# korrawe/harp

Hardware: AMD Instinct MI355X
Metric: render+loss+backward+Adam frames/sec, 512x512 MANO hand mesh (higher is better)
Workload: dtype f32; 1 GPU; C3/C4: 256-frame 512x512 sequence, subdivided MANO hand 3093v/6152f/3327uv, self-shadow, coarse+appearance terms (displacement+texture stage, VGG excluded), dense Adam; global_batch=32, sequence_frames=256, hipgraph=True

## Files before the change

### harp_amd/csrc/shade.hip

```cpp
#include "shade_common.h"

namespace {

#ifndef SHADE_TEX_SLOTS
#define SHADE_TEX_SLOTS 512
#endif
#ifndef SHADE_VTX_SLOTS
#define SHADE_VTX_SLOTS 256
#endif
#ifndef SHADE_ACC_T
#define SHADE_ACC_T double
#endif
#ifndef SHADE_OCC
#define SHADE_OCC 3
#endif
constexpr int kTexSlots = SHADE_TEX_SLOTS, kVtxSlots = SHADE_VTX_SLOTS;
constexpr int kZlW = 32, kZlH = 24;
constexpr int kTexRows = 512;
#ifndef SHADE_PRERED
#define SHADE_PRERED 19
#endif
template <int SLOTS>
__device__ __forceinline__ int sort_slots_by_row(const int* __restrict__ keys, int width, int ylo, int yhi, int* s_box, int* s_hist,
                                                 int* s_order, int* s_wsum) {
// ... 229 lines not shown
      for (int ii = -1; ii <= 1; ++ii)
        for (int jj = -1; jj <= 1; ++jj, ++k) {
          const int yy = min(max(g.iy + ii, 0), S - 1), xx = min(max(g.ix + jj, 0), S - 1);
          tapo[k] = yy * S + xx;
          sg[k] = sigmoidf((A.zl[(size_t)b * S * S + tapo[k]] - aa) * 1000.0f);
          acc += sg[k];
        }
      g.vis = acc * (1.0f / 9.0f);
    }
    const V3 amb = ld(col), dfc = ld(col + 3), spc = ld(col + 6);
    const V3 lightc = mk(amb.x + dfc.x * cosang * g.vis, amb.y + dfc.y * cosang * g.vis, amb.z + dfc.z * cosang * g.vis);
    const V3 c = mk(lightc.x * g.texel.x + spc.x, lightc.y * g.texel.y + spc.y, lightc.z * g.texel.z + spc.z);
    const float zpix = b0 * g.t.z0 + b1 * g.t.z1 + b2 * g.t.z2;
    const float zinv = (100.0f - zpix) * (1.0f / 99.0f);
    const float zmax = fmaxf(zinv, 1e-10f);
    const float wnum = __expf((zinv - zmax) * 1e4f);
    const float delta = fmaxf(__expf((1e-10f - zmax) * 1e4f), 1e-10f);
    const float denom = wnum + delta;
    if (!BWD) {
      const float rden = rcp(denom);
      out_rgb[0] = (wnum * c.x + delta * A.bg[0]) * rden;
      out_rgb[1] = (wnum * c.y + delta * A.bg[1]) * rden;
      out_rgb[2] = (wnum * c.z + delta * A.bg[2]) * rden;
      if (A.rgb) { float* r = A.rgb + o * 3; r[0] = out_rgb[0]; r[1] = out_rgb[1]; r[2] = out_rgb[2]; }
    } else {
      const float wk = wnum * rcp(denom);
      if (fused_loss) {
        const float rden = rcp(denom);
        const float o3[3] = {(wnum * c.x + delta * A.bg[0]) * rden, (wnum * c.y + delta * A.bg[1]) * rden, (wnum * c.z + delta * A.bg[2]) * rden};
        const float wl = A.l1_w[0] * A.l1_inv * l1_m;
        float gq[3];
#pragma unroll
        for (int ch = 0; ch < 3; ++ch) {
          const float d = o3[ch] * l1_m - A.l1_target[l1_to * 3 + ch] * l1_m;
          racc[16] += fabsf(d);
          gq[ch] = wl * (float)((d > 0.f) - (d < 0.f));
        }
        gc = mk(gq[0], gq[1], gq[2]);
      }
      const V3 g_c = gc * wk;
      const V3 g_tex = mk(g_c.x * lightc.x, g_c.y * lightc.y, g_c.z * lightc.z);
      const V3 g_lc = mk(g_c.x * g.texel.x, g_c.y * g.texel.y, g_c.z * g.texel.z);
      racc[0] += g_lc.x; racc[1] += g_lc.y; racc[2] += g_lc.z;
      racc[3] += g_lc.x * cosang * g.vis; racc[4] += g_lc.y * cosang * g.vis; racc[5] += g_lc.z * cosang * g.vis;
      racc[6] += g_c.x; racc[7] += g_c.y; racc[8] += g_c.z;
      const float g_dv = g_lc.x * dfc.x + g_lc.y * dfc.y + g_lc.z * dfc.z;
      const float g_vis = g_dv * cosang;
      const float g_cos = (g.cosr > 0.f) ? g_dv * g.vis : 0.f;
      float gu = 0.f, gv = 0.f;
      V3 g_m_keep = mk(0.f, 0.f, 0.f);
      gu += dot(g_tex, tdx) * (float)(A.Wt - 1);
      gv += dot(g_tex, tdy) * -(float)(A.Ht - 1);
      V3 g_p = mk(0.f, 0.f, 0.f);
      const V3 g_nn = g.lhat * g_cos, g_lhat = g.nn * g_cos;
      V3 g_ldir = (g.llen > 1e-6f) ? (g_lhat - g.lhat * dot(g.lhat, g_lhat)) * rcp(g.llen) : g_lhat * 1e6f;
      racc[9] += g_ldir.x; racc[10] += g_ldir.y; racc[11] += g_ldir.z;
      g_p = g_p - g_ldir;
      V3 g_nfin = (g.lnh > 1e-6f) ? (g_nn - g.nn * dot(g.nn, g_nn)) * rcp(g.lnh) : g_nn * 1e6f;
      V3 g_n = g_nfin;
      if (A.nmap) {
        const V3 g_np = (g.lnp > 1e-12f) ? (g_nfin - g.nhat * dot(g.nhat, g_nfin)) * rcp(g.lnp) : g_nfin * 1e12f;
        const V3 g_m = mk(-dot(g.tu, g_np), -dot(g.tv, g_np), dot(g.n, g_np));
        g_m_keep = g_m;
        gu += dot(g_m, mdx) * (float)(A.Wt - 1);
        gv += dot(g_m, mdy) * -(float)(A.Ht - 1);
        const V3 g_tu = g_np * (-g.m.x), g_tv = g_np * (-g.m.y);
        g_n = g_np * g.m.z;
        const float x = g.n.x, y = g.n.y, s = g.s, a = g.a;
        const float g_b = s * g_tu.y + g_tv.x;
        const float g_a = s * x * x * g_tu.x + y * y * g_tv.y + g_b * x * y;
        g_n.x += 2.f * s * x * a * g_tu.x - s * g_tu.z + g_b * y * a;
        g_n.y += 2.f * y * a * g_tv.y - g_tv.z + g_b * x * a;
        g_n.z += g_a * a * a;
      }
      if (!(A.debug_skip & 1)) {
        const float ax = 1.f - g.bs.wx, ay = 1.f - g.bs.wy;
        const float cw[4] = {ax * ay, g.bs.wx * ay, ax * g.bs.wy, g.bs.wx * g.bs.wy};
        const int cx[4] = {g.bs.x0, g.bs.x0 + 1, g.bs.x0, g.bs.x0 + 1}, cy[4] = {g.bs.y0, g.bs.y0, g.bs.y0 + 1, g.bs.y0 + 1};
        const bool do_t = A.g_tex != nullptr, do_n = (A.nmap != nullptr) && (A.g_nmap != nullptr);
#pragma unroll
        for (int k = 0; k < 4; ++k) {
          if (cx[k] >= A.Wt || cy[k] >= A.Ht || cw[k] == 0.f) continue;
          const int key = cy[k] * A.Wt + cx[k];
          tb_y0 = min(tb_y0, cy[k]); tb_y1 = max(tb_y1, cy[k]);
          const int slot = s_tex.find(key);
          const float vals[6] = {g_tex.x * cw[k], g_tex.y * cw[k], g_tex.z * cw[k], g_m_keep.x * cw[k], g_m_keep.y * cw[k], g_m_keep.z * cw[k]};
          if (slot >= 0) {
#pragma unroll
            for (int c = 0; c < 3; ++c) { if (do_t) s_tex.add(slot, c, vals[c]); if (do_n) s_tex.add(slot, 3 + c, vals[3 + c]); }
          } else {
#pragma unroll
            for (int c = 0; c < 3; ++c) {
              if (do_t) atomicAdd(A.g_tex + (size_t)key * 3 + c, vals[c]);
              if (do_n) atomicAdd(A.g_nmap + (size_t)key * 3 + c, vals[3 + c]);
            }
          }
        }
      }
      if (A.zl) {
        float g_zq = 0.f;
        for (int k = 0; k < 9; ++k) {
          const float d = g_vis * (1.0f / 9.0f) * sg[k] * (1.0f - sg[k]) * 1000.0f;
          if (d != 0.f) {
            zd[BWD ? k : 0] = d;
            g_zq -= d;
          }
        }
        zix = g.ix; ziy = g.iy;
        const float* R = A.light_R + 9 * b;
        g_p = g_p + mk(R[2], R[5], R[8]) * g_zq;
        racc[12] += g.p.x * g_zq; racc[13] += g.p.y * g_zq; racc[14] += g.p.z * g_zq;
        racc[15] += g_zq;
      }
      float gb0 = dot(v0, g_p) + dot(n0, g_n) + uv0x * gu + uv0y * gv;
      float gb1 = dot(v1, g_p) + dot(n1, g_n) + uv1x * gu + uv1y * gv;
      float gb2 = dot(v2, g_p) + dot(n2, g_n) + uv2x * gu + uv2y * gv;
      float gnd[9] = {0.f, 0.f, 0.f, 0.f, 0.f, 0.f, 0.f, 0.f, 0.f};
      bary_bwd(g.t, px, py, g.br, gb0, gb1, gb2, gnd);
      const float bw[3] = {b0, b1, b2};
      vidx[0] = g.i0; vidx[1] = g.i1; vidx[2] = g.i2;
#pragma unroll
      for (int k = 0; k < 3; ++k) {
        vsc[9 * k + 0] = g_p.x * bw[k]; vsc[9 * k + 1] = g_p.y * bw[k]; vsc[9 * k + 2] = g_p.z * bw[k];
        vsc[9 * k + 3] = g_n.x * bw[k]; vsc[9 * k + 4] = g_n.y * bw[k]; vsc[9 * k + 5] = g_n.z * bw[k];
        vsc[9 * k + 6] = gnd[3 * k]; vsc[9 * k + 7] = gnd[3 * k + 1]; vsc[9 * k + 8] = gnd[3 * k + 2];
      }
    }
  }
  if (BWD && A.zl && A.g_zl && !(A.debug_skip & 4)) {
    if (threadIdx.x == 0) { s_zbox[0] = 0x7fffffff; s_zbox[1] = 0x7fffffff; }
    for (int i = threadIdx.x; i < kZlW * kZlH; i += 256) s_zwin[i] = 0.0;
    __syncthreads();
    const bool has = zix > -0x40000000;
    int mx = has ? min(max(zix - 1, 0), S - 1) : 0x7fffffff, my = has ? min(max(ziy - 1, 0), S - 1) : 0x7fffffff;
#pragma unroll
    for (int o2 = 32; o2 >= 1; o2 >>= 1) { mx = min(mx, __shfl_xor(mx, o2)); my = min(my, __shfl_xor(my, o2)); }
    if (lane == 0 && mx != 0x7fffffff) { atomicMin(&s_zbox[0], mx); atomicMin(&s_zbox[1], my); }
    __syncthreads();
    const int x0 = s_zbox[0], y0 = s_zbox[1];
    float* gz = A.g_zl + (size_t)b * S * S;
    const int znt = (S + 15) >> 4;
    if (has) {
#pragma unroll
      for (int r = 0; r < 3; ++r) {
        const int yy = min(max(ziy + r - 1, 0), S - 1);
#pragma unroll
        for (int c = 0; c < 3; ++c) {
          const float d = zd[BWD ? 3 * r + c : 0];
          if (d == 0.f) continue;
          const int xx = min(max(zix + c - 1, 0), S - 1);
          const int wx = xx - x0, wy = yy - y0;
          if (wx < kZlW && wy < kZlH) atomicAdd(&s_zwin[wy * kZlW + wx], (double)d);
          else {
            atomicAdd(gz + yy * S + xx, d);
            if (A.g_zl_tiles) A.g_zl_tiles[((size_t)b * znt + (yy >> 4)) * znt + (xx >> 4)] = 1;
          }
        }
      }
    }
    __syncthreads();
    if (x0 != 0x7fffffff) {
      for (int i = threadIdx.x; i < kZlW * kZlH; i += 256) {
        const double v = s_zwin[i];
        if (v != 0.0) {
          atomicAdd(gz + (size_t)(y0 + i / kZlW) * S + x0 + (i % kZlW), (float)v);
          if (A.g_zl_tiles) A.g_zl_tiles[((size_t)b * znt + ((y0 + i / kZlW) >> 4)) * znt + ((x0 + i % kZlW) >> 4)] = 1;
        }
      }
    }
  }
  if (BWD && !(A.debug_skip & 8)) {
    bool alive = act;
    merge_same_face<27, SHADE_PRERED>(vsc, act ? f : -1, alive, lane);
    if (alive) {
      float* gvb = A.g_verts + (size_t)b * V * 3;
      float* gnb = A.g_vnormals + (size_t)b * V * 3;
      float* gdb = A.g_ndc + (size_t)b * V * 3;
#pragma unroll
      for (int k = 0; k < 3; ++k) {
        const int slot = s_acc.find(vidx[k]);
        if (slot >= 0) {
#pragma unroll
          for (int c = 0; c < 9; ++c) s_acc.add(slot, c, vsc[9 * k + c]);
        } else {
#pragma unroll
          for (int c = 0; c < 3; ++c) {
            atomicAdd(gvb + 3 * vidx[k] + c, vsc[9 * k + c]); atomicAdd(gnb + 3 * vidx[k] + c, vsc[9 * k + 3 + c]);
            atomicAdd(gdb + 3 * vidx[k] + c, vsc[9 * k + 6 + c]);
          }
        }
      }
    }
  }
  if (!BWD && A.l1_target) {
    float acc = 0.f;
    if (in_img) {
      const size_t to = ((size_t)A.l1_fid[b] * S + yi) * S + xi;
      const float m = A.l1_mask ? A.l1_mask[to] : 1.f;
      const float wk = A.l1_w[0] * A.l1_inv * m;
      if (m != 0.f) {
#pragma unroll
        for (int ch = 0; ch < 3; ++ch) {
          const float d = out_rgb[ch] * m - A.l1_target[to * 3 + ch] * m;
          acc += fabsf(d);
          if (f >= 0) A.l1_grad[o * 3 + ch] = wk * ((d > 0.f) - (d < 0.f));
        }
      } else if (f >= 0) {
        A.l1_grad[o * 3] = 0.f; A.l1_grad[o * 3 + 1] = 0.f; A.l1_grad[o * 3 + 2] = 0.f;
      }
    }
    const float sum = block_sum_256(acc, s_red);
    if (threadIdx.x == 0 && sum != 0.f) atomicAdd(A.l1_loss, sum * A.l1_inv);
  }
  }
  if (BWD && fused_loss) {
    const float sum = block_sum_256(racc[16], s_red + 16);
    if (threadIdx.x == 0 && sum != 0.f) atomicAdd(A.l1_loss, sum * A.l1_inv);
  }
  if (BWD) {
#pragma unroll
    for (int k = 0; k < 16; ++k) {
      const float s = wave_sum(racc[k]);
      if (lane == 0 && s != 0.f) atomicAdd(&s_red[k], s);
    }
    __syncthreads();
    if (threadIdx.x < 16) {
      const float s = s_red[threadIdx.x];
      const int k = threadIdx.x;
      if (s != 0.f) {
        if (k < 9) { if (A.g_colors) atomicAdd(A.g_colors + k, s); }
        else if (k < 12) { if (A.g_light_pos) atomicAdd(A.g_light_pos + 3 * b + (k - 9), s); }
        else if (k < 15) { if (A.g_light_R) atomicAdd(A.g_light_R + 9 * b + 3 * (k - 12) + 2, s); }
        else if (A.g_light_T) atomicAdd(A.g_light_T + 3 * b + 2, s);
      }
    }
    float* gvb = A.g_verts + (size_t)b * V * 3;
    float* gnb = A.g_vnormals + (size_t)b * V * 3;
    float* gdb = A.g_ndc + (size_t)b * V * 3;
    for (int i = threadIdx.x; i < kVtxSlots; i += 256) {
      const int v = s_acc.key[i];
      if (v < 0 || (A.debug_skip & 32)) continue;
#pragma unroll
      for (int c = 0; c < 3; ++c) {
        const float a0 = (float)s_acc.val[i][c], a1 = (float)s_acc.val[i][3 + c], a2 = (float)s_acc.val[i][6 + c];
        if (a0 != 0.f) atomicAdd(gvb + 3 * v + c, a0);
        if (a1 != 0.f) atomicAdd(gnb + 3 * v + c, a1);
        if (a2 != 0.f) atomicAdd(gdb + 3 * v + c, a2);
      }
    }
    __shared__ int s_box[2];
    __shared__ int s_wsum[4];
    static_assert(sizeof(double) * kZlW * kZlH >= sizeof(int) * (kTexRows + kTexSlots), "window too small for the sort scratch");
    int* s_hist = (int*)s_zwin;
    int* s_order = s_hist + kTexRows;
    if (!(A.debug_skip & 16)) {
      const int total = sort_slots_by_row<kTexSlots>(s_tex.key, A.Wt, tb_y0, tb_y1, s_box, s_hist, s_order, s_wsum);
      if (total >= 0) {
        for (int i = threadIdx.x; i < total * 3; i += 256) {
          const int e = i / 3, c = i - 3 * e;
          const int slot = s_order[e];
          const int key = s_tex.key[slot];
          const float a0 = (float)s_tex.val[slot][c], a1 = (float)s_tex.val[slot][3 + c];
          if (a0 != 0.f) atomicAdd(A.g_tex + (size_t)key * 3 + c, a0);
          if (a1 != 0.f) atomicAdd(A.g_nmap + (size_t)key * 3 + c, a1);
        }
      } else {
        for (int i = threadIdx.x; i < kTexSlots; i += 256) {
          const int key = s_tex.key[i];
          if (key < 0) continue;
#pragma unroll
          for (int c = 0; c < 3; ++c) {
            const float a0 = (float)s_tex.val[i][c], a1 = (float)s_tex.val[i][3 + c];
            if (a0 != 0.f) atomicAdd(A.g_tex + (size_t)key * 3 + c, a0);
            if (a1 != 0.f) atomicAdd(A.g_nmap + (size_t)key * 3 + c, a1);
          }
        }
      }
    }
  }
}

__global__ void pack_texels_kernel(const float* __restrict__ tex, const float* __restrict__ nmap, int n, float4* __restrict__ out) {
  const int i = blockIdx.x * blockDim.x + threadIdx.x;
  if (i >= n) return;
  out[2 * i] = make_float4(tex[3 * i], tex[3 * i + 1], tex[3 * i + 2], nmap[3 * i]);
  out[2 * i + 1] = make_float4(nmap[3 * i + 1], nmap[3 * i + 2], 0.f, 0.f);
}
__global__ void normalize_pack_kernel(const float* __restrict__ tex, const float* __restrict__ nmap_raw, int n, float* __restrict__ nmap_n,
                                      float4* __restrict__ out) {
  const int i = blockIdx.x * blockDim.x + threadIdx.x;
  if (i >= n) return;
  float n0, n1, n2;
  normalize3_texel(nmap_raw[3 * i], nmap_raw[3 * i + 1], nmap_raw[3 * i + 2], n0, n1, n2);
  nmap_n[3 * i] = n0; nmap_n[3 * i + 1] = n1; nmap_n[3 * i + 2] = n2;
  if (out) {
    out[2 * i] = make_float4(tex[3 * i], tex[3 * i + 1], tex[3 * i + 2], n0);
    out[2 * i + 1] = make_float4(n1, n2, 0.f, 0.f);
  }
}

struct NmapBwd {
  const float* x; const float* gy; float* gx; int n; int blocks;
  float* v9; float* gv; float* gn; float* gd; int nv; int v9_blocks;
};
__device__ __forceinline__ void vert9_unpack_body(float* __restrict__ g9, float* __restrict__ gv, float* __restrict__ gn, float* __restrict__ gd,
                                                  int nv, size_t first, size_t stride) {
  for (size_t i = first; i < (size_t)nv * 9; i += stride) {
    const float x = g9[i];
    if (x != 0.f) {
      const size_t v = i / 9;
      const int c = (int)(i - 9 * v);
      float* dst = c < 3 ? gv : (c < 6 ? gn : gd);
      atomicAdd(dst + 3 * v + (c % 3), x);
      g9[i] = 0.f;
    }
  }
}
__global__ void __launch_bounds__(256) vert9_unpack_kernel(float* __restrict__ g9, float* __restrict__ gv, float* __restrict__ gn, float* __restrict__ gd, int nv) {
  vert9_unpack_body(g9, gv, gn, gd, nv, (size_t)blockIdx.x * 256 + threadIdx.x, (size_t)gridDim.x * 256);
}
template <bool CONSUME, bool NMAP = false>
__global__ void __launch_bounds__(256) depth_bwd_kernel(const int32_t* __restrict__ face_id, const FaceRec* __restrict__ recs,
                                                        const int32_t* __restrict__ faces, float* __restrict__ g_z,
                                                        int V, int F, int S, float* __restrict__ g_ndc,
                                                        const int32_t* __restrict__ order, const int32_t* __restrict__ nact,
                                                        int B, int nsx, const NmapBwd M, unsigned char* __restrict__ tiles) {
  __shared__ VertexAccum<256, 3> s_acc;
  const unsigned tile_blocks = NMAP ? gridDim.x - (unsigned)M.blocks - (unsigned)M.v9_blocks : gridDim.x;
  if (NMAP && blockIdx.x >= tile_blocks) {
    const unsigned e = blockIdx.x - tile_blocks;
    if (e < (unsigned)M.blocks) {
      for (size_t i = (size_t)e * 256 + threadIdx.x; i < (size_t)M.n; i += (size_t)M.blocks * 256) normalize3_bwd_texel(M.x, M.gy, M.gx, i);
    } else {
      vert9_unpack_body(M.v9, M.gv, M.gn, M.gd, M.nv, (size_t)(e - M.blocks) * 256 + threadIdx.x, (size_t)M.v9_blocks * 256);
    }
    return;
  }
  const unsigned limit = (unsigned)(((nact[0] + 7) / 8) * 8 * (kSuper / kTile) * (kSuper / kTile));
  for (unsigned vb = blockIdx.x; vb < limit; vb += tile_blocks) {
  if (vb != blockIdx.x) __syncthreads();
  int b, st, tx0, ty0, tsub;
  if (tile_decode_v(vb, order, nact, B, nsx, S, b, st, tx0, ty0, tsub, false) != 1) continue;
  if (tiles) {
    const int znt = (S + 15) >> 4;
    unsigned char* fl = tiles + ((size_t)b * znt + (ty0 >> 4)) * znt + (tx0 >> 4);
    if (*fl == 0) continue;
    __syncthreads();
    if (threadIdx.x == 0) *fl = 0;
  }
  const int lane = threadIdx.x & 63, w = threadIdx.x >> 6;
  const int xi = tx0 + (lane & 15), yi = ty0 + w * 4 + (lane >> 4);
  const bool in_img = xi < S && yi < S;
  const size_t o = ((size_t)b * S + (in_img ? yi : 0)) * S + (in_img ? xi : 0);
  const int f = in_img ? face_id[o] : -1;
  const float g = in_img ? g_z[o] : 0.f;
  if (CONSUME && g != 0.f) g_z[o] = 0.f;
  const bool act = f >= 0 && g != 0.f;
  if (__syncthreads_or(act ? 1 : 0) == 0) continue;
  s_acc.clear();
  __syncthreads();
  float* gdb = g_ndc + (size_t)b * V * 3;
  float gnd[9] = {0.f, 0.f, 0.f, 0.f, 0.f, 0.f, 0.f, 0.f, 0.f};
  if (act) {
    const Tri t = load_tri(recs + (size_t)b * F + f);
    const float px = pix_to_ndc(xi, S), py = pix_to_ndc(yi, S);
    const Bary br = bary_fwd(t, px, py);
    gnd[2] = g * br.b0; gnd[5] = g * br.b1; gnd[8] = g * br.b2;
    bary_bwd(t, px, py, br, g * t.z0, g * t.z1, g * t.z2, gnd);
  }
  bool alive = act;
  merge_same_face<9, SHADE_PRERED>(gnd, act ? f : -1, alive, lane);
  if (alive) {
    const int vi[3] = {faces[3 * f], faces[3 * f + 1], faces[3 * f + 2]};
#pragma unroll
    for (int k = 0; k < 3; ++k) {
      const int slot = s_acc.find(vi[k]);
#pragma unroll
      for (int c = 0; c < 3; ++c) {
        if (slot >= 0) s_acc.add(slot, c, gnd[3 * k + c]); else atomicAdd(gdb + 3 * vi[k] + c, gnd[3 * k + c]);
      }
    }
  }
  __syncthreads();
  for (int i = threadIdx.x; i < 256; i += 256) {
    const int v = s_acc.key[i];
    if (v < 0) continue;
#pragma unroll
    for (int c = 0; c < 3; ++c) if (s_acc.val[i][c] != 0) atomicAdd(gdb + 3 * v + c, (float)s_acc.val[i][c]);
  }
  }
}

}

int harp_detail_shade_bwd_wave(const harp_shade_args& a, const int32_t* order, const int32_t* nact, int nsx, unsigned grid, hipStream_t stream);
int harp_detail_fused_bwd(const harp_shade_args& a, const void* ws, const int32_t* faces, float blur, float sigma, const float* alpha,
                          const float* g_alpha, hipStream_t stream);

extern "C" {

int harp_pack_texels(const float* tex, const float* nmap, int n_texels, float* out, hipStream_t stream) {
  if (!tex || !nmap || !out || n_texels <= 0) return HARP_ERR_ARG;
  hipLaunchKernelGGL(pack_texels_kernel, dim3((n_texels + 255) / 256), dim3(256), 0, stream, tex, nmap, n_texels, (float4*)out);
  HARP_CHECK_LAUNCH();
  return HARP_OK;
}

int harp_shade_fwd(const harp_shade_args* a, hipStream_t stream) {
  if (!a || !a->face_id || !a->recs || !a->faces || !a->faces_uvs || !a->verts_uvs || !a->verts || !a->vnormals || !a->tex ||
      !a->light_pos || !a->colors || (!a->rgb && !a->l1_target) || (a->zl && (!a->light_R || !a->light_T)))
    return HARP_ERR_ARG;
  const RasterWs W = raster_ws_split((void*)a->recs, a->B, a->F, a->S);
  const dim3 grid(tile_grid(a->B, W.nsx));
  harp_shade_args b = *a;
  if (b.l1_target) {
    if (!b.l1_fid || !b.l1_w || !b.l1_loss || !b.l1_grad) return HARP_ERR_ARG;
    b.l1_inv = 1.0f / ((float)b.B * (float)b.S * (float)b.S * 3.0f);
  }
  hipLaunchKernelGGL(shade_kernel<false>, grid, dim3(256), 0, stream, b, (const int32_t*)W.order, (const int32_t*)W.nact, W.nsx);
  HARP_CHECK_LAUNCH();
  return HARP_OK;
}

int harp_shade_bwd(const harp_shade_args* a, hipStream_t stream) {
  if (!a || !a->face_id || !a->recs) return HARP_ERR_ARG;
  const bool geom = a->g_verts && a->g_vnormals && a->g_ndc;
  if (!geom && (a->g_verts || a->g_vnormals || a->g_ndc || (a->debug_skip & 0xff))) return HARP_ERR_ARG;
  harp_shade_args b = *a;
  if (!b.g_rgb) {
    if (!b.l1_target || !b.l1_fid || !b.l1_w || !b.l1_loss || !b.l1_bg_sums) return HARP_ERR_ARG;
    b.l1_inv = 1.0f / ((float)b.B * (float)b.S * (float)b.S * 3.0f);
  } else {
    b.l1_target = nullptr;
  }
  if (b.g_vert9 && (!geom || (b.debug_skip & 0xff))) return HARP_ERR_ARG;
  if (b.trec && (!b.trec_cnt || b.trec_cap <= 0 || (b.trec_cap & 3) || (b.g_tex && !b.trec_acc_tex) || (b.nmap && b.g_nmap && !b.trec_acc_nmap) || (b.debug_skip & 0xff) || b.Wt > 65535 || b.Ht > 65535)) return HARP_ERR_ARG;
  const RasterWs W = raster_ws_split((void*)a->recs, a->B, a->F, a->S);
  if ((b.debug_skip & 0xff) == 0) return harp_detail_shade_bwd_wave(b, (const int32_t*)W.order, (const int32_t*)W.nact, W.nsx, tile_grid(a->B, W.nsx), stream);
  hipLaunchKernelGGL(shade_kernel<true>, dim3(tile_grid(a->B, W.nsx)), dim3(256), 0, stream, b, (const int32_t*)W.order, (const int32_t*)W.nact, W.nsx);
  HARP_CHECK_LAUNCH();
  return HARP_OK;
}

int harp_shade_sil_bwd(const harp_shade_args* a, float blur_radius, float sigma, const float* alpha, const float* g_alpha, hipStream_t stream) {
  if (!a || !a->face_id || !a->recs || !a->faces || !a->g_verts || !a->g_vnormals || !a->g_ndc || !alpha || !g_alpha) return HARP_ERR_ARG;
  harp_shade_args b = *a;
  if (!b.g_rgb) {
    if (!b.l1_target || !b.l1_fid || !b.l1_w || !b.l1_loss || !b.l1_bg_sums) return HARP_ERR_ARG;
    b.l1_inv = 1.0f / ((float)b.B * (float)b.S * (float)b.S * 3.0f);
  } else {
    b.l1_target = nullptr;
  }
  b.debug_skip = 0;
  b.trec = nullptr;
  return harp_detail_fused_bwd(b, a->recs, a->faces, blur_radius, sigma, alpha, g_alpha, stream);
}

int harp_depth_bwd(const int32_t* face_id, const void* ws, const int32_t* faces, const float* g_z, int B, int V, int F, int S,
                   float* g_ndc, hipStream_t stream) {
  if (!face_id || !ws || !faces || !g_z || !g_ndc) return HARP_ERR_ARG;
  const RasterWs W = raster_ws_split((void*)ws, B, F, S);
  hipLaunchKernelGGL(depth_bwd_kernel<false>, dim3(min(tile_grid(B, W.nsx), 4096u)), dim3(256), 0, stream, face_id, (const FaceRec*)ws, faces, (float*)g_z, V, F, S,
                     g_ndc, (const int32_t*)W.order, (const int32_t*)W.nact, B, W.nsx, NmapBwd{}, nullptr);
  HARP_CHECK_LAUNCH();
  return HARP_OK;
}

int harp_depth_bwd_consume(const int32_t* face_id, const void* ws, const int32_t* faces, float* g_z, int B, int V, int F, int S,
                           float* g_ndc, hipStream_t stream) {
  if (!face_id || !ws || !faces || !g_z || !g_ndc) return HARP_ERR_ARG;
  const RasterWs W = raster_ws_split((void*)ws, B, F, S);
  hipLaunchKernelGGL(depth_bwd_kernel<true>, dim3(min(tile_grid(B, W.nsx), 4096u)), dim3(256), 0, stream, face_id, (const FaceRec*)ws, faces, g_z, V, F, S, g_ndc,
                     (const int32_t*)W.order, (const int32_t*)W.nact, B, W.nsx, NmapBwd{}, nullptr);
  HARP_CHECK_LAUNCH();
  return HARP_OK;
}

int harp_depth_bwd_tiles(const int32_t* face_id, const void* ws, const int32_t* faces, float* g_z, int B, int V, int F, int S,
                         float* g_ndc, unsigned char* g_z_tiles, hipStream_t stream) {
  if (!face_id || !ws || !faces || !g_z || !g_ndc) return HARP_ERR_ARG;
  const RasterWs W = raster_ws_split((void*)ws, B, F, S);
  hipLaunchKernelGGL(depth_bwd_kernel<true>, dim3(min(tile_grid(B, W.nsx), 4096u)), dim3(256), 0, stream, face_id, (const FaceRec*)ws, faces, g_z, V, F, S, g_ndc,
                     (const int32_t*)W.order, (const int32_t*)W.nact, B, W.nsx, NmapBwd{}, g_z_tiles);
  HARP_CHECK_LAUNCH();
  return HARP_OK;
}

int harp_depth_nmap_bwd(const int32_t* face_id, const void* ws, const int32_t* faces, float* g_z, int B, int V, int F, int S, float* g_ndc,
                        const float* nmap, const float* g_nmap_n, int n_texels, float* g_nmap, unsigned char* g_z_tiles, hipStream_t stream) {
  if (!face_id || !ws || !faces || !g_z || !g_ndc || !nmap || !g_nmap_n || !g_nmap || n_texels <= 0) return HARP_ERR_ARG;
  const RasterWs W = raster_ws_split((void*)ws, B, F, S);
  const NmapBwd M{nmap, g_nmap_n, g_nmap, n_texels, min((n_texels + 255) / 256, 1024), nullptr, nullptr, nullptr, nullptr, 0, 0};
  hipLaunchKernelGGL((depth_bwd_kernel<true, true>), dim3(min(tile_grid(B, W.nsx), 4096u) + (unsigned)M.blocks), dim3(256), 0, stream, face_id,
                     (const FaceRec*)ws, faces, g_z, V, F, S, g_ndc, (const int32_t*)W.order, (const int32_t*)W.nact, B, W.nsx, M, g_z_tiles);
  HARP_CHECK_LAUNCH();
  return HARP_OK;
}

int harp_depth_bwd_riders(const int32_t* face_id, const void* ws, const int32_t* faces, float* g_z, int B, int V, int F, int S, float* g_ndc,
                          unsigned char* g_z_tiles, const float* nmap, const float* g_nmap_n, int n_texels, float* g_nmap, float* g_vert9,
                          float* g_verts, float* g_vnormals, float* g_ndc_cam, hipStream_t stream) {
  if (!face_id || !ws || !faces || !g_z || !g_ndc) return HARP_ERR_ARG;
  if (nmap && (!g_nmap_n || !g_nmap || n_texels <= 0)) return HARP_ERR_ARG;
  if (g_vert9 && (!g_verts || !g_vnormals || !g_ndc_cam)) return HARP_ERR_ARG;
  const RasterWs W = raster_ws_split((void*)ws, B, F, S);
  NmapBwd M{nmap, g_nmap_n, g_nmap, nmap ? n_texels : 0, nmap ? min((n_texels + 255) / 256, 1024) : 0,
            g_vert9, g_verts, g_vnormals, g_ndc_cam, g_vert9 ? B * V : 0, g_vert9 ? min((B * V * 9 + 255) / 256, 1024) : 0};
  hipLaunchKernelGGL((depth_bwd_kernel<true, true>), dim3(min(tile_grid(B, W.nsx), 4096u) + (unsigned)M.blocks + (unsigned)M.v9_blocks), dim3(256), 0, stream,
                     face_id, (const FaceRec*)ws, faces, g_z, V, F, S, g_ndc, (const int32_t*)W.order, (const int32_t*)W.nact, B, W.nsx, M, g_z_tiles);
  HARP_CHECK_LAUNCH();
  return HARP_OK;
}

int harp_vert9_unpack(float* g_vert9, int n_verts, float* g_verts, float* g_vnormals, float* g_ndc, hipStream_t stream) {
  if (!g_vert9 || !g_verts || !g_vnormals || !g_ndc || n_verts <= 0) return HARP_ERR_ARG;
  hipLaunchKernelGGL(vert9_unpack_kernel, dim3(min((n_verts * 9 + 255) / 256, 1024)), dim3(256), 0, stream, g_vert9, g_verts, g_vnormals, g_ndc, n_verts);
  HARP_CHECK_LAUNCH();
  return HARP_OK;
}

int harp_normalize3_pack(const float* tex, const float* nmap_raw, int n_texels, float* nmap_n, float* packed, hipStream_t stream) {
  if (!nmap_raw || !nmap_n || n_texels <= 0 || (packed && !tex)) return HARP_ERR_ARG;
  const char* e = getenv("HARP_SIDE_LDS");
  hipLaunchKernelGGL(normalize_pack_kernel, dim3((n_texels + 255) / 256), dim3(256), e ? (size_t)atoi(e) : 512, stream, tex, nmap_raw, n_texels, nmap_n, (float4*)packed);
  HARP_CHECK_LAUNCH();
  return HARP_OK;
}

}
```

### harp_amd/csrc/texel_reduce.hip

```cpp
#include <stdlib.h>
#include "harp_common.h"
#include "harp_hip.h"

namespace {

constexpr int kBin = 32;
constexpr int kAcc = kBin + 1;
constexpr int kChunk = 2048;
constexpr int kThreads = 512;
constexpr int kMaxBins = 1024;

__device__ __forceinline__ void fixed_scale40(float m, double& s, double& inv) {
  int e = ((__float_as_int(m) >> 23) & 0xff) - 126;
  e = min(max(e, -100), 100);
  s = __longlong_as_double((long long)(1023 + 40 - e) << 52);
  inv = __longlong_as_double((long long)(1023 - 40 + e) << 52);
}
__device__ __forceinline__ long long to_fixed(double x) {
  return __double_as_longlong(x + 6755399441055744.0) - 0x4338000000000000ll;
}

__global__ void __launch_bounds__(kThreads) texel_reduce_kernel(const float* __restrict__ rec, int32_t* __restrict__ cnt, int cap, int nbins, int nbx,
                                                                int Wt, int Ht, double* __restrict__ g_tex, double* __restrict__ g_nmap) {
  __shared__ long long acc[2][kAcc * kAcc * 3];
  __shared__ float wmax[2][kThreads / 64];
  __shared__ int pre[kMaxBins];
  __shared__ int cl[kMaxBins];
  __shared__ int wsum[kThreads / 64];
  const int t = threadIdx.x, lane = t & 63, w = t >> 6;
  int carry = 0;
  for (int b0 = 0; b0 < nbins; b0 += kThreads) {
    const int b = b0 + t;
    const int c = b < nbins ? min(cnt[16 * b], cap) : 0;
    int v = (c + kChunk - 1) / kChunk;
#pragma unroll
    for (int d = 1; d < 64; d <<= 1) { const int o = __shfl_up(v, d, 64); if (lane >= d) v += o; }
    if (lane == 63) wsum[w] = v;
    __syncthreads();
    int off = carry;
    for (int i = 0; i < w; ++i) off += wsum[i];
    if (b < nbins) { pre[b] = v + off; cl[b] = c; }
    int tot = 0;
    for (int i = 0; i < kThreads / 64; ++i) tot += wsum[i];
    carry += tot;
    __syncthreads();
  }
  const int total = carry;
  for (int chunk = blockIdx.x; chunk < total; chunk += gridDim.x) {
    int lo = 0, hi = nbins - 1;
    while (lo < hi) { const int mid = (lo + hi) >> 1; if (pre[mid] > chunk) hi = mid; else lo = mid + 1; }
    const int bin = lo;
    const int first = (chunk - (bin ? pre[bin - 1] : 0)) * kChunk;
    const int n = min(cl[bin] - first, kChunk);
    for (int i = t; i < 2 * kAcc * kAcc * 3; i += kThreads) (&acc[0][0])[i] = 0;
    const float* r0 = rec + (size_t)bin * 9 * (size_t)cap + (size_t)first;
    const size_t capz = (size_t)cap;
    float rv[kChunk / kThreads][9];
    static_assert(kChunk / kThreads == 4, "one float4 per plane and thread");
    {
      const int i = 4 * t;
      if (i < n) {
#pragma unroll
        for (int k = 0; k < 9; ++k) {
          const float4 q = *(const float4*)(r0 + k * capz + i);
          rv[0][k] = q.x; rv[1][k] = q.y; rv[2][k] = q.z; rv[3][k] = q.w;
        }
      }
    }
    float m0 = 0.f, m1 = 0.f;
#pragma unroll
    for (int j = 0; j < kChunk / kThreads; ++j) {
      if (4 * t + j < n) {
        m0 = fmaxf(m0, fmaxf(fabsf(rv[j][3]), fmaxf(fabsf(rv[j][4]), fabsf(rv[j][5]))));
        m1 = fmaxf(m1, fmaxf(fabsf(rv[j][6]), fmaxf(fabsf(rv[j][7]), fabsf(rv[j][8]))));
      }
    }
    m0 = wave_max_u(m0); m1 = wave_max_u(m1);
    if (lane == 0) { wmax[0][w] = m0; wmax[1][w] = m1; }
    __syncthreads();
#pragma unroll
    for (int i = 0; i < kThreads / 64; ++i) { m0 = fmaxf(m0, wmax[0][i]); m1 = fmaxf(m1, wmax[1][i]); }
    double s0, i0, s1, i1;
    fixed_scale40(m0, s0, i0);
    fixed_scale40(m1, s1, i1);
#pragma unroll
    for (int j = 0; j < kChunk / kThreads; ++j) {
      const int i = 4 * t + j;
      if (i < n) {
        const int key = __float_as_int(rv[j][0]);
        const int x0 = key & 0xffff, y0 = (int)((unsigned)key >> 16);
        const float wx = rv[j][1], wy = rv[j][2];
        const float ax = 1.f - wx, ay = 1.f - wy;
        const float cw[4] = {ax * ay, wx * ay, ax * wy, wx * wy};
        const int lx = x0 & (kBin - 1), ly = y0 & (kBin - 1);
#pragma unroll
        for (int k = 0; k < 4; ++k) {
          const int cx = x0 + (k & 1), cy = y0 + (k >> 1);
          if (cx < Wt && cy < Ht && cw[k] != 0.f) {
            const int o = ((ly + (k >> 1)) * kAcc + lx + (k & 1)) * 3;
#pragma unroll
            for (int c = 0; c < 3; ++c) {
              if (g_tex) atomicAdd((unsigned long long*)&acc[0][o + c], (unsigned long long)to_fixed((double)(rv[j][3 + c] * cw[k]) * s0));
              if (g_nmap) atomicAdd((unsigned long long*)&acc[1][o + c], (unsigned long long)to_fixed((double)(rv[j][6 + c] * cw[k]) * s1));
            }
          }
        }
      }
    }
    __syncthreads();
    const int bx = bin % nbx, by = bin / nbx;
    for (int i = t; i < kAcc * kAcc * 3; i += kThreads) {
      const int ly = i / (kAcc * 3), q = i - ly * (kAcc * 3);
      const int gx3 = bx * kBin * 3 + q, gy = by * kBin + ly;
      if (gy < Ht && gx3 < Wt * 3) {
        const size_t o = (size_t)gy * Wt * 3 + gx3;
        const long long a0 = acc[0][i], a1 = acc[1][i];
        if (g_tex && a0 != 0) atomicAdd(g_tex + o, (double)a0 * i0);
        if (g_nmap && a1 != 0) atomicAdd(g_nmap + o, (double)a1 * i1);
      }
    }
    __syncthreads();
  }
}

__global__ void __launch_bounds__(256) texel_finish_kernel(double* __restrict__ acc_tex, float* __restrict__ g_tex, double* __restrict__ acc_nmap,
                                                           float* __restrict__ g_nmap, const float* __restrict__ nmap_raw, int n) {
  const int i = blockIdx.x * 256 + threadIdx.x;
  if (i >= n) return;
  if (acc_tex) {
    const double a = acc_tex[3 * (size_t)i], b = acc_tex[3 * (size_t)i + 1], c = acc_tex[3 * (size_t)i + 2];
    if (a != 0.0 || b != 0.0 || c != 0.0) {
      g_tex[3 * (size_t)i] += (float)a; g_tex[3 * (size_t)i + 1] += (float)b; g_tex[3 * (size_t)i + 2] += (float)c;
      acc_tex[3 * (size_t)i] = 0.0; acc_tex[3 * (size_t)i + 1] = 0.0; acc_tex[3 * (size_t)i + 2] = 0.0;
    }
  }
  if (acc_nmap) {
    const double a = acc_nmap[3 * (size_t)i], b = acc_nmap[3 * (size_t)i + 1], c = acc_nmap[3 * (size_t)i + 2];
    if (a != 0.0 || b != 0.0 || c != 0.0) {
      acc_nmap[3 * (size_t)i] = 0.0; acc_nmap[3 * (size_t)i + 1] = 0.0; acc_nmap[3 * (size_t)i + 2] = 0.0;
      if (nmap_raw) {
        normalize3_bwd_vals(nmap_raw, (float)a, (float)b, (float)c, g_nmap, (size_t)i);
      } else {
        g_nmap[3 * (size_t)i] += (float)a; g_nmap[3 * (size_t)i + 1] += (float)b; g_nmap[3 * (size_t)i + 2] += (float)c;
      }
    }
  }
}

__global__ void texel_counters_clear_kernel(int32_t* __restrict__ cnt, int nbins) {
  for (int b = threadIdx.x; b < nbins; b += blockDim.x) cnt[16 * b] = 0;
}

}

extern "C" {

int harp_texel_bins(int Ht, int Wt) { return (Ht <= 0 || Wt <= 0) ? 0 : ((Ht + kBin - 1) / kBin) * ((Wt + kBin - 1) / kBin); }

int harp_texel_reduce(const float* trec, int32_t* trec_cnt, int trec_cap, int Ht, int Wt, double* acc_tex, double* acc_nmap, int expected_records,
                      hipStream_t stream) {
  const int nbins = harp_texel_bins(Ht, Wt);
  if (!trec || !trec_cnt || trec_cap <= 0 || (trec_cap & 3) || ((size_t)trec & 15) || nbins <= 0 || nbins > kMaxBins || Wt > 65535 || Ht > 65535) return HARP_ERR_ARG;
  const bool small_job = expected_records <= 2000000;
  const unsigned grid = small_job ? 256u : 512u;
  const size_t pad = small_job ? 21504 : 12288;
  hipLaunchKernelGGL(texel_reduce_kernel, dim3(grid), dim3(kThreads), pad, stream, trec, trec_cnt, trec_cap, nbins, (Wt + kBin - 1) / kBin, Wt, Ht, acc_tex, acc_nmap);
  hipLaunchKernelGGL(texel_counters_clear_kernel, dim3(1), dim3(256), 0, stream, trec_cnt, nbins);
  HARP_CHECK_LAUNCH();
  return HARP_OK;
}

int harp_texel_finish(double* acc_tex, float* g_tex, double* acc_nmap, float* g_nmap, const float* nmap_raw, int n_texels, hipStream_t stream) {
  if (n_texels <= 0 || (acc_tex && !g_tex) || (acc_nmap && !g_nmap) || (!acc_tex && !acc_nmap)) return HARP_ERR_ARG;
  hipLaunchKernelGGL(texel_finish_kernel, dim3((n_texels + 255) / 256), dim3(256), 0, stream, acc_tex, g_tex, acc_nmap, g_nmap, nmap_raw, n_texels);
  HARP_CHECK_LAUNCH();
  return HARP_OK;
}

}
```

Baseline: 53550 frames/s.

## Prefetch next tile/chunk in depth and texel backward reductions, merge adjacent texel atomics

```diff
diff --git a/harp_amd/csrc/shade.hip b/harp_amd/csrc/shade.hip
--- a/harp_amd/csrc/shade.hip
+++ b/harp_amd/csrc/shade.hip
@@ -555,6 +555,7 @@
 struct NmapBwd {
   const float* x; const float* gy; float* gx; int n; int blocks;
   float* v9; float* gv; float* gn; float* gd; int nv; int v9_blocks;
+  int lead;
 };
 __device__ __forceinline__ void vert9_unpack_body(float* __restrict__ g9, float* __restrict__ gv, float* __restrict__ gn, float* __restrict__ gd,
                                                   int nv, size_t first, size_t stride) {
@@ -579,37 +580,55 @@
                                                         const int32_t* __restrict__ order, const int32_t* __restrict__ nact,
                                                         int B, int nsx, const NmapBwd M, unsigned char* __restrict__ tiles) {
   __shared__ VertexAccum<256, 3> s_acc;
-  const unsigned tile_blocks = NMAP ? gridDim.x - (unsigned)M.blocks - (unsigned)M.v9_blocks : gridDim.x;
-  if (NMAP && blockIdx.x >= tile_blocks) {
-    const unsigned e = blockIdx.x - tile_blocks;
+  const unsigned lead = NMAP ? (unsigned)M.lead : 0u;
+  const unsigned tile_blocks = gridDim.x - lead;
+  if (NMAP && blockIdx.x < lead) {
+    const unsigned e = blockIdx.x;
     if (e < (unsigned)M.blocks) {
       for (size_t i = (size_t)e * 256 + threadIdx.x; i < (size_t)M.n; i += (size_t)M.blocks * 256) normalize3_bwd_texel(M.x, M.gy, M.gx, i);
-    } else {
+    } else if (e < (unsigned)M.blocks + (unsigned)M.v9_blocks) {
       vert9_unpack_body(M.v9, M.gv, M.gn, M.gd, M.nv, (size_t)(e - M.blocks) * 256 + threadIdx.x, (size_t)M.v9_blocks * 256);
     }
     return;
   }
-  const unsigned limit = (unsigned)(((nact[0] + 7) / 8) * 8 * (kSuper / kTile) * (kSuper / kTile));
-  for (unsigned vb = blockIdx.x; vb < limit; vb += tile_blocks) {
-  if (vb != blockIdx.x) __syncthreads();
-  int b, st, tx0, ty0, tsub;
-  if (tile_decode_v(vb, order, nact, B, nsx, S, b, st, tx0, ty0, tsub, false) != 1) continue;
-  if (tiles) {
-    const int znt = (S + 15) >> 4;
-    unsigned char* fl = tiles + ((size_t)b * znt + (ty0 >> 4)) * znt + (tx0 >> 4);
-    if (*fl == 0) continue;
-    __syncthreads();
-    if (threadIdx.x == 0) *fl = 0;
-  }
+  const unsigned bid0 = blockIdx.x - lead;
+  const int nact0 = nact[0];
+  const unsigned limit = (unsigned)(((nact0 + 7) / 8) * 8 * (kSuper / kTile) * (kSuper / kTile));
   const int lane = threadIdx.x & 63, w = threadIdx.x >> 6;
-  const int xi = tx0 + (lane & 15), yi = ty0 + w * 4 + (lane >> 4);
-  const bool in_img = xi < S && yi < S;
-  const size_t o = ((size_t)b * S + (in_img ? yi : 0)) * S + (in_img ? xi : 0);
-  const int f = in_img ? face_id[o] : -1;
-  const float g = in_img ? g_z[o] : 0.f;
+  const int znt = (S + 15) >> 4;
+  struct Req { int ok, b, tx0, ty0, flag, f; float g; };
+  auto pixel = [&](const Req& r, int& xi, int& yi) -> size_t {
+    xi = r.tx0 + (lane & 15); yi = r.ty0 + w * 4 + (lane >> 4);
+    const bool in_img = xi < S && yi < S;
+    return ((size_t)r.b * S + (in_img ? yi : 0)) * S + (in_img ? xi : 0);
+  };
+  auto flag_of = [&](const Req& r) { return tiles + ((size_t)r.b * znt + (r.ty0 >> 4)) * znt + (r.tx0 >> 4); };
+  auto request = [&](unsigned vb) -> Req {
+    Req r;
+    r.ok = 0; r.b = 0; r.tx0 = 0; r.ty0 = 0; r.flag = 1; r.f = -1; r.g = 0.f;
+    int st, tsub;
+    if (vb >= limit || tile_decode_v(vb, order, nact, B, nsx, S, r.b, st, r.tx0, r.ty0, tsub, false) != 1) return r;
+    int xi, yi;
+    const size_t o = pixel(r, xi, yi);
+    if (tiles) r.flag = __builtin_amdgcn_readfirstlane((int)*flag_of(r));
+    if (xi < S && yi < S) { r.f = face_id[o]; r.g = g_z[o]; }
+    r.ok = 1;
+    return r;
+  };
+  Req nx = request(bid0);
+  for (unsigned vb = bid0; vb < limit; vb += tile_blocks) {
+  const Req cu = nx;
+  nx = request(vb + tile_blocks);
+  if (!cu.ok || cu.flag == 0) continue;
+  const int b = cu.b, f = cu.f;
+  const float g = cu.g;
+  int xi, yi;
+  const size_t o = pixel(cu, xi, yi);
   if (CONSUME && g != 0.f) g_z[o] = 0.f;
   const bool act = f >= 0 && g != 0.f;
-  if (__syncthreads_or(act ? 1 : 0) == 0) continue;
+  const int any = __syncthreads_or(act ? 1 : 0);
+  if (tiles && threadIdx.x == 0) *flag_of(cu) = 0;
+  if (any == 0) continue;
   s_acc.clear();
   __syncthreads();
   float* gdb = g_ndc + (size_t)b * V * 3;
@@ -709,11 +728,15 @@
   return harp_detail_fused_bwd(b, a->recs, a->faces, blur_radius, sigma, alpha, g_alpha, stream);
 }
 
+static unsigned depth_bwd_grid(int B, int nsx) { return min(tile_grid(B, nsx), 4096u); }
+
+static int riders_lead(int riders) { return (riders + 7) & ~7; }
+
 int harp_depth_bwd(const int32_t* face_id, const void* ws, const int32_t* faces, const float* g_z, int B, int V, int F, int S,
                    float* g_ndc, hipStream_t stream) {
   if (!face_id || !ws || !faces || !g_z || !g_ndc) return HARP_ERR_ARG;
   const RasterWs W = raster_ws_split((void*)ws, B, F, S);
-  hipLaunchKernelGGL(depth_bwd_kernel<false>, dim3(min(tile_grid(B, W.nsx), 4096u)), dim3(256), 0, stream, face_id, (const FaceRec*)ws, faces, (float*)g_z, V, F, S,
+  hipLaunchKernelGGL(depth_bwd_kernel<false>, dim3(depth_bwd_grid(B, W.nsx)), dim3(256), 0, stream, face_id, (const FaceRec*)ws, faces, (float*)g_z, V, F, S,
                      g_ndc, (const int32_t*)W.order, (const int32_t*)W.nact, B, W.nsx, NmapBwd{}, nullptr);
   HARP_CHECK_LAUNCH();
   return HARP_OK;
@@ -723,7 +746,7 @@
                            float* g_ndc, hipStream_t stream) {
   if (!face_id || !ws || !faces || !g_z || !g_ndc) return HARP_ERR_ARG;
   const RasterWs W = raster_ws_split((void*)ws, B, F, S);
-  hipLaunchKernelGGL(depth_bwd_kernel<true>, dim3(min(tile_grid(B, W.nsx), 4096u)), dim3(256), 0, stream, face_id, (const FaceRec*)ws, faces, g_z, V, F, S, g_ndc,
+  hipLaunchKernelGGL(depth_bwd_kernel<true>, dim3(depth_bwd_grid(B, W.nsx)), dim3(256), 0, stream, face_id, (const FaceRec*)ws, faces, g_z, V, F, S, g_ndc,
                      (const int32_t*)W.order, (const int32_t*)W.nact, B, W.nsx, NmapBwd{}, nullptr);
   HARP_CHECK_LAUNCH();
   return HARP_OK;
@@ -733,7 +756,7 @@
                          float* g_ndc, unsigned char* g_z_tiles, hipStream_t stream) {
   if (!face_id || !ws || !faces || !g_z || !g_ndc) return HARP_ERR_ARG;
   const RasterWs W = raster_ws_split((void*)ws, B, F, S);
-  hipLaunchKernelGGL(depth_bwd_kernel<true>, dim3(min(tile_grid(B, W.nsx), 4096u)), dim3(256), 0, stream, face_id, (const FaceRec*)ws, faces, g_z, V, F, S, g_ndc,
+  hipLaunchKernelGGL(depth_bwd_kernel<true>, dim3(depth_bwd_grid(B, W.nsx)), dim3(256), 0, stream, face_id, (const FaceRec*)ws, faces, g_z, V, F, S, g_ndc,
                      (const int32_t*)W.order, (const int32_t*)W.nact, B, W.nsx, NmapBwd{}, g_z_tiles);
   HARP_CHECK_LAUNCH();
   return HARP_OK;
@@ -743,8 +766,9 @@
                         const float* nmap, const float* g_nmap_n, int n_texels, float* g_nmap, unsigned char* g_z_tiles, hipStream_t stream) {
   if (!face_id || !ws || !faces || !g_z || !g_ndc || !nmap || !g_nmap_n || !g_nmap || n_texels <= 0) return HARP_ERR_ARG;
   const RasterWs W = raster_ws_split((void*)ws, B, F, S);
-  const NmapBwd M{nmap, g_nmap_n, g_nmap, n_texels, min((n_texels + 255) / 256, 1024), nullptr, nullptr, nullptr, nullptr, 0, 0};
-  hipLaunchKernelGGL((depth_bwd_kernel<true, true>), dim3(min(tile_grid(B, W.nsx), 4096u) + (unsigned)M.blocks), dim3(256), 0, stream, face_id,
+  NmapBwd M{nmap, g_nmap_n, g_nmap, n_texels, min((n_texels + 255) / 256, 1024), nullptr, nullptr, nullptr, nullptr, 0, 0, 0};
+  M.lead = riders_lead(M.blocks);
+  hipLaunchKernelGGL((depth_bwd_kernel<true, true>), dim3(depth_bwd_grid(B, W.nsx) + (unsigned)M.lead), dim3(256), 0, stream, face_id,
                      (const FaceRec*)ws, faces, g_z, V, F, S, g_ndc, (const int32_t*)W.order, (const int32_t*)W.nact, B, W.nsx, M, g_z_tiles);
   HARP_CHECK_LAUNCH();
   return HARP_OK;
@@ -758,8 +782,9 @@
   if (g_vert9 && (!g_verts || !g_vnormals || !g_ndc_cam)) return HARP_ERR_ARG;
   const RasterWs W = raster_ws_split((void*)ws, B, F, S);
   NmapBwd M{nmap, g_nmap_n, g_nmap, nmap ? n_texels : 0, nmap ? min((n_texels + 255) / 256, 1024) : 0,
-            g_vert9, g_verts, g_vnormals, g_ndc_cam, g_vert9 ? B * V : 0, g_vert9 ? min((B * V * 9 + 255) / 256, 1024) : 0};
-  hipLaunchKernelGGL((depth_bwd_kernel<true, true>), dim3(min(tile_grid(B, W.nsx), 4096u) + (unsigned)M.blocks + (unsigned)M.v9_blocks), dim3(256), 0, stream,
+            g_vert9, g_verts, g_vnormals, g_ndc_cam, g_vert9 ? B * V : 0, g_vert9 ? min((B * V * 9 + 255) / 256, 1024) : 0, 0};
+  M.lead = riders_lead(M.blocks + M.v9_blocks);
+  hipLaunchKernelGGL((depth_bwd_kernel<true, true>), dim3(depth_bwd_grid(B, W.nsx) + (unsigned)M.lead), dim3(256), 0, stream,
                      face_id, (const FaceRec*)ws, faces, g_z, V, F, S, g_ndc, (const int32_t*)W.order, (const int32_t*)W.nact, B, W.nsx, M, g_z_tiles);
   HARP_CHECK_LAUNCH();
   return HARP_OK;
diff --git a/harp_amd/csrc/texel_reduce.hip b/harp_amd/csrc/texel_reduce.hip
--- a/harp_amd/csrc/texel_reduce.hip
+++ b/harp_amd/csrc/texel_reduce.hip
@@ -20,13 +20,36 @@
   return __double_as_longlong(x + 6755399441055744.0) - 0x4338000000000000ll;
 }
 
+#ifndef HARP_TEXEL_PITCH
+#define HARP_TEXEL_PITCH 40
+#endif
+constexpr int kPitch = HARP_TEXEL_PITCH;
+constexpr int kPlane = kAcc * kPitch;
+constexpr int kStaticLds = 6 * kPlane * 8 + 2 * (kThreads / 64) * 4 + 2 * kMaxBins * 4 + (kThreads / 64) * 4;
+static_assert(kPitch >= kAcc, "a table row holds 33 texels");
+
+#ifndef HARP_TEXEL_PREFETCH
+#define HARP_TEXEL_PREFETCH 9
+#endif
+constexpr int kPrefetch = HARP_TEXEL_PREFETCH;
+template <int K0, int K1>
+__device__ __forceinline__ void load_records(const float* __restrict__ r0, size_t capz, int t, int n, float (&rv)[4][9]) {
+  const int i = 4 * t < n ? 4 * t : 0;
+#pragma unroll
+  for (int k = K0; k < K1; ++k) {
+    const float4 q = *(const float4*)(r0 + k * capz + i);
+    rv[0][k] = q.x; rv[1][k] = q.y; rv[2][k] = q.z; rv[3][k] = q.w;
+  }
+}
+
 __global__ void __launch_bounds__(kThreads) texel_reduce_kernel(const float* __restrict__ rec, int32_t* __restrict__ cnt, int cap, int nbins, int nbx,
                                                                 int Wt, int Ht, double* __restrict__ g_tex, double* __restrict__ g_nmap) {
-  __shared__ long long acc[2][kAcc * kAcc * 3];
+  __shared__ long long acc[6][kPlane];
   __shared__ float wmax[2][kThreads / 64];
   __shared__ int pre[kMaxBins];
   __shared__ int cl[kMaxBins];
   __shared__ int wsum[kThreads / 64];
+  static_assert(sizeof(acc) + sizeof(wmax) + sizeof(pre) + sizeof(cl) + sizeof(wsum) == kStaticLds, "the launch pads are sized from kStaticLds");
   const int t = threadIdx.x, lane = t & 63, w = t >> 6;
   int carry = 0;
   for (int b0 = 0; b0 < nbins; b0 += kThreads) {
@@ -46,27 +69,22 @@
     __syncthreads();
   }
   const int total = carry;
-  for (int chunk = blockIdx.x; chunk < total; chunk += gridDim.x) {
+  const size_t capz = (size_t)cap;
+  auto locate = [&](int chunk, int& bin, int& n, int& first) -> const float* {
     int lo = 0, hi = nbins - 1;
     while (lo < hi) { const int mid = (lo + hi) >> 1; if (pre[mid] > chunk) hi = mid; else lo = mid + 1; }
-    const int bin = lo;
-    const int first = (chunk - (bin ? pre[bin - 1] : 0)) * kChunk;
-    const int n = min(cl[bin] - first, kChunk);
-    for (int i = t; i < 2 * kAcc * kAcc * 3; i += kThreads) (&acc[0][0])[i] = 0;
-    const float* r0 = rec + (size_t)bin * 9 * (size_t)cap + (size_t)first;
-    const size_t capz = (size_t)cap;
-    float rv[kChunk / kThreads][9];
-    static_assert(kChunk / kThreads == 4, "one float4 per plane and thread");
-    {
-      const int i = 4 * t;
-      if (i < n) {
-#pragma unroll
-        for (int k = 0; k < 9; ++k) {
-          const float4 q = *(const float4*)(r0 + k * capz + i);
-          rv[0][k] = q.x; rv[1][k] = q.y; rv[2][k] = q.z; rv[3][k] = q.w;
-        }
-      }
-    }
+    bin = __builtin_amdgcn_readfirstlane(lo);
+    first = __builtin_amdgcn_readfirstlane((chunk - (bin ? pre[bin - 1] : 0)) * kChunk);
+    n = __builtin_amdgcn_readfirstlane(min(cl[bin] - first, kChunk));
+    return rec + (size_t)bin * 9 * capz + (size_t)first;
+  };
+  float rv[kChunk / kThreads][9];
+  static_assert(kChunk / kThreads == 4, "one float4 per plane and thread");
+  int bin = 0, n = 0, first = 0;
+  if ((int)blockIdx.x < total) load_records<0, kPrefetch>(locate(blockIdx.x, bin, n, first), capz, t, n, rv);
+  for (int chunk = blockIdx.x; chunk < total; chunk += gridDim.x) {
+    if (kPrefetch < 9) load_records<kPrefetch, 9>(rec + (size_t)bin * 9 * capz + (size_t)first, capz, t, n, rv);
+    for (int i = t; i < 6 * kPlane; i += kThreads) (&acc[0][0])[i] = 0;
     float m0 = 0.f, m1 = 0.f;
 #pragma unroll
     for (int j = 0; j < kChunk / kThreads; ++j) {
@@ -80,46 +98,94 @@
     __syncthreads();
 #pragma unroll
     for (int i = 0; i < kThreads / 64; ++i) { m0 = fmaxf(m0, wmax[0][i]); m1 = fmaxf(m1, wmax[1][i]); }
+    m0 = __int_as_float(__builtin_amdgcn_readfirstlane(__float_as_int(m0)));
+    m1 = __int_as_float(__builtin_amdgcn_readfirstlane(__float_as_int(m1)));
     double s0, i0, s1, i1;
     fixed_scale40(m0, s0, i0);
     fixed_scale40(m1, s1, i1);
-#pragma unroll
-    for (int j = 0; j < kChunk / kThreads; ++j) {
-      const int i = 4 * t + j;
-      if (i < n) {
-        const int key = __float_as_int(rv[j][0]);
-        const int x0 = key & 0xffff, y0 = (int)((unsigned)key >> 16);
-        const float wx = rv[j][1], wy = rv[j][2];
-        const float ax = 1.f - wx, ay = 1.f - wy;
-        const float cw[4] = {ax * ay, wx * ay, ax * wy, wx * wy};
-        const int lx = x0 & (kBin - 1), ly = y0 & (kBin - 1);
-#pragma unroll
-        for (int k = 0; k < 4; ++k) {
-          const int cx = x0 + (k & 1), cy = y0 + (k >> 1);
-          if (cx < Wt && cy < Ht && cw[k] != 0.f) {
-            const int o = ((ly + (k >> 1)) * kAcc + lx + (k & 1)) * 3;
+    float nv[kChunk / kThreads][9];
+    int nbin = 0, nn = 0, nfirst = 0;
+    if (chunk + (int)gridDim.x < total) load_records<0, kPrefetch>(locate(chunk + gridDim.x, nbin, nn, nfirst), capz, t, nn, nv);
+    float cwm[4][4];
+    int off[4];
+    bool same[4], right[4], left[4], live[4];
+#pragma unroll
+    for (int j = 0; j < 4; ++j) {
+      const int key = __float_as_int(rv[j][0]);
+      const int x0 = key & 0xffff, y0 = (int)((unsigned)key >> 16);
+      live[j] = 4 * t + j < n;
+      const float wx = rv[j][1], wy = rv[j][2];
+      const float ax = 1.f - wx, ay = 1.f - wy;
+      const float cw[4] = {ax * ay, wx * ay, ax * wy, wx * wy};
+#pragma unroll
+      for (int k = 0; k < 4; ++k) cwm[j][k] = (live[j] && x0 + (k & 1) < Wt && y0 + (k >> 1) < Ht) ? cw[k] : 0.f;
+      off[j] = (y0 & (kBin - 1)) * kPitch + (x0 & (kBin - 1));
+      same[j] = right[j] = left[j] = false;
+      if (j > 0) {
+        const int d = key - __float_as_int(rv[j - 1][0]);
+        same[j] = live[j] && d == 0; right[j] = live[j] && d == 1; left[j] = live[j] && d == -1;
+      }
+    }
+#pragma unroll
+    for (int map = 0; map < 2; ++map) {
+      if (map == 0 ? g_tex == nullptr : g_nmap == nullptr) continue;
+      const double s = map == 0 ? s0 : s1;
+      long long pend[3][4];
+#pragma unroll
+      for (int j = 0; j <= 4; ++j) {
+        if (j > 0) {
+          const bool sm = j < 4 && same[j], rt = j < 4 && right[j], lf = j < 4 && left[j];
+#pragma unroll
+          for (int k = 0; k < 4; ++k) {
+            const bool keep = sm || ((k & 1) ? rt : lf);
+            if (live[j - 1] && !keep) {
+#pragma unroll
+              for (int c = 0; c < 3; ++c) {
+                atomicAdd((unsigned long long*)&acc[3 * map + c][off[j - 1] + (k >> 1) * kPitch + (k & 1)], (unsigned long long)pend[c][k]);
+              }
+            }
+          }
+          if (j < 4) {
 #pragma unroll
             for (int c = 0; c < 3; ++c) {
-              if (g_tex) atomicAdd((unsigned long long*)&acc[0][o + c], (unsigned long long)to_fixed((double)(rv[j][3 + c] * cw[k]) * s0));
-              if (g_nmap) atomicAdd((unsigned long long*)&acc[1][o + c], (unsigned long long)to_fixed((double)(rv[j][6 + c] * cw[k]) * s1));
+              const long long q0 = pend[c][0], q1 = pend[c][1], q2 = pend[c][2], q3 = pend[c][3];
+              pend[c][0] = sm ? q0 : (rt ? q1 : 0);
+              pend[c][1] = sm ? q1 : (lf ? q0 : 0);
+              pend[c][2] = sm ? q2 : (rt ? q3 : 0);
+              pend[c][3] = sm ? q3 : (lf ? q2 : 0);
             }
           }
         }
+        if (j < 4) {
+#pragma unroll
+          for (int c = 0; c < 3; ++c)
+#pragma unroll
+            for (int k = 0; k < 4; ++k) {
+              const long long v = to_fixed((double)(rv[j][3 + 3 * map + c] * cwm[j][k]) * s);
+              pend[c][k] = j == 0 ? v : pend[c][k] + v;
+            }
+        }
       }
     }
     __syncthreads();
     const int bx = bin % nbx, by = bin / nbx;
     for (int i = t; i < kAcc * kAcc * 3; i += kThreads) {
       const int ly = i / (kAcc * 3), q = i - ly * (kAcc * 3);
+      const int lx = q / 3, c = q - 3 * lx;
       const int gx3 = bx * kBin * 3 + q, gy = by * kBin + ly;
       if (gy < Ht && gx3 < Wt * 3) {
         const size_t o = (size_t)gy * Wt * 3 + gx3;
-        const long long a0 = acc[0][i], a1 = acc[1][i];
+        const long long a0 = acc[c][ly * kPitch + lx], a1 = acc[3 + c][ly * kPitch + lx];
         if (g_tex && a0 != 0) atomicAdd(g_tex + o, (double)a0 * i0);
         if (g_nmap && a1 != 0) atomicAdd(g_nmap + o, (double)a1 * i1);
       }
     }
     __syncthreads();
+#pragma unroll
+    for (int j = 0; j < 4; ++j)
+#pragma unroll
+      for (int k = 0; k < kPrefetch; ++k) rv[j][k] = nv[j][k];
+    bin = nbin; n = nn; first = nfirst;
   }
 }
 
@@ -163,7 +229,7 @@
   if (!trec || !trec_cnt || trec_cap <= 0 || (trec_cap & 3) || ((size_t)trec & 15) || nbins <= 0 || nbins > kMaxBins || Wt > 65535 || Ht > 65535) return HARP_ERR_ARG;
   const bool small_job = expected_records <= 2000000;
   const unsigned grid = small_job ? 256u : 512u;
-  const size_t pad = small_job ? 21504 : 12288;
+  const size_t pad = (small_job ? 82064 : 72848) - kStaticLds;
   hipLaunchKernelGGL(texel_reduce_kernel, dim3(grid), dim3(kThreads), pad, stream, trec, trec_cnt, trec_cap, nbins, (Wt + kBin - 1) / kBin, Wt, Ht, acc_tex, acc_nmap);
   hipLaunchKernelGGL(texel_counters_clear_kernel, dim3(1), dim3(256), 0, stream, trec_cnt, nbins);
   HARP_CHECK_LAUNCH();
```

Result: no change. 53930 frames/s, median of 3 (+0.7%).
